# edwinyosorahardjo/compressjs-flattened

Hardware: AMD Instinct MI355X
Metric: bzip2 -9 compress MB/s at 1/2/4/8 MI355X; bit-exact output size vs ref (higher is better)
Workload: dtype u32; 1 GPU; Bzip2.compressFile level 9 (899981-byte blocks) on 1 x 100000000 bytes enwik8-shaped synthetic text (tools/textgen.c seed 1), device-resident; per_gpu_bytes=100000000, level=9, parallelism=1 GPU

## Files before the change

### compressjs-flattened_amd/csrc/bwt.hip

```cpp
#include "cjs_internal.h"
#include "prims.hpp"
#include <stdlib.h>
#include <string.h>

namespace cjs {

struct Geom { uint32_t nb, stride, n_last; };
__device__ __forceinline__ uint32_t blk_len(const Geom& g, uint32_t blk) { return blk == g.nb - 1 ? g.n_last : g.stride; }
struct VarGeom { uint32_t nb, stride, n_last; const uint32_t* len; };
__device__ __forceinline__ uint32_t blk_len(const VarGeom& g, uint32_t blk) { return g.len[blk]; }
template <typename G> struct is_var_geom { static constexpr bool value = false; };
template <> struct is_var_geom<VarGeom> { static constexpr bool value = true; };

__device__ __forceinline__ uint32_t xcd_tile(uint32_t wg, uint32_t T) {
  const uint32_t per = (T + 7u) >> 3;
  return (wg & 7u) * per + (wg >> 3);
}
__host__ __device__ __forceinline__ uint32_t xcd_grid(uint32_t T) { return ((T + 7u) >> 3) << 3; }

struct SegGeom { uint32_t nseg, stride, n_last, tps; };
struct TileRef { uint32_t seg, off, nvalid; uint64_t base; };
__device__ __forceinline__ TileRef tile_ref(const SegGeom& sg, uint32_t tile) {
  TileRef t;
  t.seg = tile / sg.tps;
// ... 351 lines not shown
    uint32_t any = 0;
    for (int j = 0; j < 8; j++) any |= hword[threadIdx.x * 8 + j];
    if (!any) atomicOr(big_flag, 1u);
  }
  surv = block_sum<256>(surv, sm);
  heads = block_sum<256>(heads, sm);
  last = wave_max(last);
  if (lane_id() == 0) sm[wave_id()] = last;
  __syncthreads();
  if (threadIdx.x == 0) {
    uint32_t m = sm[0]; for (int i = 1; i < 4; i++) m = sm[i] > m ? sm[i] : m;
    tile_cnt[blockIdx.x] = surv; tile_cnt[T + blockIdx.x] = heads; tile_cnt[2 * (size_t)T + blockIdx.x] = m;
  }
}

__global__ __launch_bounds__(1024) void bwt_scan_tiles(uint32_t* __restrict__ tile_cnt, uint32_t T, uint32_t* __restrict__ counters,
                                                      uint32_t* __restrict__ host_mirror ) {
  __shared__ uint32_t sm[16];
  __shared__ uint32_t mx[1024];
  uint32_t c0 = 0, c1 = 0, cm = 0;
  for (uint32_t base = 0; base < T; base += 1024) {
    const uint32_t i = base + threadIdx.x;
    const bool ok = i < T;
    uint32_t t0, t1;
    const uint32_t v0 = ok ? tile_cnt[i] : 0u, v1 = ok ? tile_cnt[T + i] : 0u, v2 = ok ? tile_cnt[2 * (size_t)T + i] : 0u;
    const uint32_t e0 = block_excl_sum<1024>(v0, sm, t0);
    const uint32_t e1 = block_excl_sum<1024>(v1, sm, t1);
    const uint32_t im = block_incl_max<1024>(v2, sm);
    mx[threadIdx.x] = im;
    __syncthreads();
// ... 21 lines not shown
  uint64_t lo = seg0, hi = base - 64u;
  while (hi > lo) {
    const uint64_t len = hi - lo, step = (len + 63u) / 64u, idx = lo + (uint64_t)lane * step;
    const bool hit = idx >= hi || (key[idx] >> shift) == target;
    const uint64_t hits = __ballot(hit);
    const uint32_t j = hits ? (uint32_t)__builtin_ctzll(hits) : 64u;
    if (!j) { hi = lo; break; }
    const uint64_t nhi = lo + (uint64_t)j * step;
    lo += (uint64_t)(j - 1u) * step + 1u;
    if (j < 64u && nhi < hi) hi = nhi;
  }
  return hi;
}

template <bool FIRST, bool PACKED, int SWEEP = 0, typename G = Geom>
__global__ __launch_bounds__(256) void bwt_apply(const uint64_t* __restrict__ key, const uint32_t* __restrict__ val,
                                                 const uint32_t* __restrict__ pos, uint32_t A, G g,
                                                 uint32_t* tile_cnt, uint32_t T,
                                                 uint32_t* __restrict__ R, uint32_t* __restrict__ SA,
                                                 uint32_t* __restrict__ nval, uint32_t* __restrict__ npos, uint32_t* __restrict__ ngord, HalfMap hm_,
                                                 const uint8_t* __restrict__ Tx, uint8_t* __restrict__ U, uint32_t* __restrict__ big_flag,
                                                 int gs1 , int carried ) {
  __shared__ uint64_t sk[RS_TILE + 2];
  __shared__ uint64_t m_nh[64], m_sg[64], m_oh[64];
  __shared__ uint32_t wp_s[64], wp_h[64], wp_head[64];
  __shared__ uint32_t carry_s;
  const uint32_t tile = xcd_tile(blockIdx.x, T), half = SWEEP == 2 ? 1u : 0u;
  if (tile >= T) return;
  const uint32_t hsplit = hm_.stride >> 1;
  const int tid = threadIdx.x, w = tid >> 6, lane = tid & 63;
  const uint64_t base = (uint64_t)tile * RS_TILE;
  const uint32_t nvalid = (uint32_t)((uint64_t)A - base < RS_TILE ? (uint64_t)A - base : RS_TILE);
  uint32_t sbase = 0, hbase = 0, carry = 0;
  if (SWEEP != 1) { sbase = tile_cnt[tile]; hbase = tile_cnt[T + tile]; carry = tile_cnt[2 * (size_t)T + tile]; }
  else if (w == 0) {
    const uint64_t seg0 = (uint64_t)((uint32_t)base / g.stride) * g.stride;
    const uint32_t c = (uint32_t)class_head_before(key, seg0, base, gs1, lane) + 1u;
    if (lane == 0) carry_s = c;
  }
  uint32_t p16[FIRST ? 1 : 16], v16[PACKED ? 1 : 16];
  {
    uint64_t k16[16];
#pragma unroll
    for (int it = 0; it < 16; it++) {
      const uint32_t e = (uint32_t)it * 256u + tid;
      k16[it] = __builtin_nontemporal_load(key + base + (e < nvalid ? e : nvalid - 1u));
    }
    if (!FIRST) {
#pragma unroll
      for (int it = 0; it < 16; it++) { const uint32_t e = (uint32_t)it * 256u + tid; p16[it] = __builtin_nontemporal_load(pos + base + (e < nvalid ? e : nvalid - 1u)); }
    }
    if (!PACKED) {
#pragma unroll
      for (int it = 0; it < 16; it++) { const uint32_t e = (uint32_t)it * 256u + tid; v16[it] = __builtin_nontemporal_load(val + base + (e < nvalid ? e : nvalid - 1u)); }
    }
    if (tid == 0) sk[0] = base ? key[base - 1] : ~0ull;
    if (tid == 64) sk[RS_TILE + 1] = base + RS_TILE < A ? key[base + RS_TILE] : ~0ull;
#pragma unroll
    for (int it = 0; it < 16; it++) {
      const uint32_t e = (uint32_t)it * 256u + tid;
      sk[e + 1] = e < nvalid ? k16[it] : ~0ull;
    }
  }
  __syncthreads();
  const int GS = FIRST ? gs1 : 0;
  const uint64_t bnd = FIRST ? (base + g.stride - 1u) / g.stride * g.stride : ~0ull;
#pragma unroll 4
  for (int it = 0; it < 16; it++) {
    const uint32_t e = (uint32_t)it * 256u + tid;
    const uint64_t a = base + e;
    const bool ok = e < nvalid;
    const uint64_t k = sk[e + 1] >> GS;
    const bool nh = ok && (a == 0 || a == bnd || (sk[e] >> GS) != k);
    const bool nx = a + 1 == A || a + 1 == bnd || (sk[e + 2] >> GS) != k;
    const uint64_t mnh = __ballot(nh), msg = __ballot(nh && nx);
    if (lane == 0) { m_nh[it * 4 + w] = mnh; m_sg[it * 4 + w] = msg; }
    if (!FIRST) {
      const bool oh = ok && (a == 0 || (sk[e] >> 20) != (sk[e + 1] >> 20));
      const uint64_t moh = __ballot(oh);
      if (lane == 0) m_oh[it * 4 + w] = moh;
    }
  }
  __syncthreads();
  if (w == 0) {
    const uint64_t mh = m_nh[lane], ms = m_sg[lane];
    const uint32_t first = (uint32_t)lane * 64u;
    const uint32_t nv = nvalid > first ? (nvalid - first < 64u ? nvalid - first : 64u) : 0u;
    const uint64_t vm = nv == 64 ? ~0ull : ((1ull << nv) - 1ull);
    const uint32_t sv = (uint32_t)__popcll(vm & ~ms), hd = (uint32_t)__popcll(mh & ~ms);
    const uint32_t lastrel = mh ? first + 63u - (uint32_t)__builtin_clzll(mh) + 1u : 0u;
    const uint32_t is = wave_incl_sum(sv), ih = wave_incl_sum(hd), im = wave_incl_max(lastrel);
    uint32_t em = __shfl_up(im, 1, 64);
    if (lane == 0) em = 0;
    wp_s[lane] = is - sv; wp_h[lane] = ih - hd; wp_head[lane] = em;
    if (SWEEP == 1 && lane == 63) {
      tile_cnt[tile] = is; tile_cnt[T + tile] = ih; tile_cnt[2 * (size_t)T + tile] = im ? (uint32_t)base + im : 0u;
    }
    if (SWEEP == 1) {
      const uint64_t nz = __ballot(mh != 0);
      bool bad = false;
#pragma unroll
      for (int b = 0; b < 8; b++) bad |= base + (uint64_t)(b + 1) * 512u <= A && ((nz >> (8 * b)) & 0xFFull) == 0;
      if (bad && lane == 0) atomicOr(big_flag, 1u);
// ... 21 lines not shown
  for (int it = 0; it < 16; it++) {
    const uint32_t e = (uint32_t)it * 256u + tid;
    if (e < nvalid) {
      const uint64_t a = base + e;
      const int wi = it * 4 + w;
      const uint64_t mh = m_nh[wi], ms = m_sg[wi];
      const uint64_t hm = mh & le;
      uint32_t head_a;
      bool keeps_rank = false;
      if (hm || wp_head[wi]) {
        const uint32_t hrel = hm ? (uint32_t)wi * 64u + 63u - (uint32_t)__builtin_clzll(hm) : wp_head[wi] - 1u;
        head_a = (uint32_t)base + hrel;
        if (!FIRST) keeps_rank = (m_oh[hrel >> 6] >> (hrel & 63u)) & 1ull;
      } else {
        head_a = carry - 1u;
        if (!FIRST) keeps_rank = head_a == 0 || (key[head_a] >> 20) != (key[head_a - 1] >> 20);
      }
      const uint32_t p = FIRST ? (uint32_t)a : p16[FIRST ? 0 : it];
      const uint32_t vraw = PACKED ? (uint32_t)sk[e + 1] : v16[PACKED ? 0 : it];
      const uint32_t vv = vraw & PK_POS_MASK;
      const uint32_t pb = PACKED ? (vraw >> PK2_PREV_SHIFT) & 0xFFu : vraw >> VAL_PREV_SHIFT;
      const uint32_t blk = p / g.stride;
      const uint32_t head_pos = p - ((uint32_t)a - head_a);
      if (!keeps_rank && (SWEEP == 0 || (uint32_t)(vv >= hsplit) == half)) R[(size_t)blk * g.stride + vv] = head_pos - blk * g.stride;
      if (SWEEP == 1) continue;
      if ((ms >> lane) & 1ull) {
        if (U) U[p] = (uint8_t)(carried ? pb : ub[it]);
        else __builtin_nontemporal_store(vv, SA + p);
      } else {
        const uint32_t so = sbase + wp_s[wi] + (uint32_t)__popcll(~ms & lt);
        const uint32_t ho = hbase + wp_h[wi] + (uint32_t)__popcll(mh & ~ms & le);
// ... 51 lines not shown
    else if (j >= n) { j = 0; past |= 1u << s; }
    pp[s] = blk * tg.g.stride + j;
  }
#pragma unroll
  for (int s = 0; s < 16; s++) rk20[s] = tg.R[((need >> s) & 1u) ? pp[s] : pp[0]];
#pragma unroll
  for (int s = 0; s < 16; s++) rk20[s] = ((past >> s) & 1u) ? 0u : rk20[s] + 1u;
}

__device__ __forceinline__ void ts_ce(uint64_t& a, uint64_t& b, bool up) {
  const bool sw = (a > b) == up;
  const uint64_t x = sw ? b : a, y = sw ? a : b;
  a = x; b = y;
}
template <typename TG>
__global__ __launch_bounds__(256) void bwt_tile_sort(uint64_t* __restrict__ key, uint32_t* __restrict__ val, uint32_t A,
                                                     uint8_t* __restrict__ dflag, TG tg, uint32_t Tt) {
  __shared__ uint64_t sk[TS_WIN];
  __shared__ uint64_t hm[64];
  __shared__ int32_t wlast[64], wnext[64];
  uint32_t* gk = (uint32_t*)sk;
  const int tid = threadIdx.x, w = tid >> 6, lane = tid & 63;
  __shared__ uint32_t lired[4];
  const uint32_t win = xcd_tile(blockIdx.x, Tt);
  if (win >= Tt) return;
  const uint64_t wb = (uint64_t)win * TS_NOM;
  const uint64_t we = (wb + TS_WIN < A) ? wb + TS_WIN : A;
  const uint32_t L = (uint32_t)(we - wb);
  uint64_t r[16];
  uint32_t pv[16], go[16], pp[16];
  uint32_t gprev;
// ... 69 lines not shown
    }
  }
  __syncthreads();
  uint32_t* sk32 = reinterpret_cast<uint32_t*>(sk);
#pragma unroll
  for (int it = 0; it < 16; it++) { const uint32_t x = (uint32_t)it * 256u + tid; sk32[x] = ((uint32_t)(r[it] >> 32) << 12) | x; }
  any_medium = __syncthreads_or(any_medium);
#pragma unroll
  for (int it = 0; it < 16; it++) {
    const bool own = hx16[it] != 0xFFFFFFFFu && (hx16[it] >> 16) <= TS_TINY;
    const uint32_t hx = own ? (hx16[it] & 0xFFFFu) : 0u, g = own ? (hx16[it] >> 16) : 0u;
    const uint32_t gmax = wave_max(g);
    if (gmax == 0) continue;
    const uint64_t mine = r[it];
    const uint32_t mine32 = ((uint32_t)(mine >> 32) << 12) | ((uint32_t)it * 256u + tid);
    uint32_t rank = 0;
    for (uint32_t d = 0; d < gmax; d++) rank += (d < g && sk32[hx + d] < mine32) ? 1u : 0u;
    if (own) {
      key[wb + hx + rank] = ((uint64_t)go[it] << 20) | ((mine >> 32) & 0xFFFFFull);
      val[wb + hx + rank] = (uint32_t)mine;
    }
  }
  if (!any_medium) return;
  if (w == 0) {
    const uint32_t pc = (uint32_t)__builtin_popcountll(mm[lane]);
    const uint32_t inc = wave_incl_sum(pc);
    mpre[lane] = inc - pc;
    if (lane == 63) mpre[64] = inc;
  }
  __syncthreads();
  const uint32_t Mt = mpre[64];
  uint32_t P = 2;
  while (P < Mt) P <<= 1;
  uint32_t cix[16];
// ... 24 lines not shown
      const uint32_t hj = j >> 1;
      for (uint32_t t = tid; t < (P >> 2); t += 256) {
        const uint32_t i0 = ((t & ~(hj - 1)) << 2) | (t & (hj - 1));
        const bool up = (i0 & kk) == 0;
        uint64_t e0 = sk[i0], e1 = sk[i0 | hj], e2 = sk[i0 | j], e3 = sk[i0 | j | hj];
        ts_ce(e0, e2, up); ts_ce(e1, e3, up); ts_ce(e0, e1, up); ts_ce(e2, e3, up);
        sk[i0] = e0; sk[i0 | hj] = e1; sk[i0 | j] = e2; sk[i0 | j | hj] = e3;
      }
      __syncthreads();
    }
  }
#pragma unroll
  for (int it = 0; it < 16; it++) {
    if (cix[it] != 0xFFFFFFFFu) {
      const uint32_t x = (uint32_t)it * 256u + tid;
      const uint64_t e = sk[cix[it]];
      key[wb + x] = ((uint64_t)go[it] << 20) | ((e >> 32) & 0xFFFFFull);
      val[wb + x] = (uint32_t)e;
    }
  }
}
template <typename TG>
__global__ __launch_bounds__(256) void bwt_tile_sort_radix(uint64_t* __restrict__ key, uint32_t* __restrict__ val, uint32_t A,
                                                           uint8_t* __restrict__ dflag, TG tg, uint32_t Tt) {
  __shared__ uint64_t se[TS_WIN];
  __shared__ uint64_t hm[64];
  __shared__ int32_t wlast[64], wnext[64];
  __shared__ uint32_t wcnt[4][256];
  __shared__ uint32_t sm[4];
  uint32_t* gk = (uint32_t*)se;
  const int tid = threadIdx.x, w = tid >> 6, lane = tid & 63;
  __shared__ uint32_t lired[4];
  const uint32_t win = xcd_tile(blockIdx.x, Tt);
  if (win >= Tt) return;
  const uint64_t wb = (uint64_t)win * TS_NOM;
  const uint64_t we = (wb + TS_WIN < A) ? wb + TS_WIN : A;
  const uint32_t L = (uint32_t)(we - wb);
  uint32_t rk20[16], go[16], pv[16], pp[16];
// ... 82 lines not shown
      const uint32_t d = (comp[s] >> shift) & 255u;
      se[wcnt[w][d] + rk[s]] = ((uint64_t)comp[s] << 32) | pv[s];
    }
    __syncthreads();
#pragma unroll
    for (int s = 0; s < 16; s++) {
      const uint64_t e = se[(uint32_t)w * 1024u + (uint32_t)s * 64u + lane];
      comp[s] = (uint32_t)(e >> 32); pv[s] = (uint32_t)e;
    }
    __syncthreads();
  }
#pragma unroll
  for (int s = 0; s < 16; s++) {
    if ((ownm >> s) & 1u) {
      const uint32_t x = (uint32_t)w * 1024u + (uint32_t)s * 64u + lane;
      key[wb + x] = ((uint64_t)go[s] << 20) | (comp[s] & 0xFFFFFu);
      val[wb + x] = pv[s];
    }
  }
}
__global__ __launch_bounds__(1024) void scan_u32_single(uint32_t* __restrict__ arr, uint32_t n, uint32_t* __restrict__ total, uint32_t* __restrict__ host_total) {
  __shared__ uint32_t sm[16];
  uint32_t carry = 0;
  for (uint32_t base = 0; base < n; base += 1024) {
    const uint32_t i = base + threadIdx.x;
    uint32_t v = i < n ? arr[i] : 0u, tot;
    const uint32_t ex = block_excl_sum<1024>(v, sm, tot);
    if (i < n) arr[i] = carry + ex;
    carry += tot;
  }
  if (threadIdx.x == 0) { *total = carry; *host_total = carry; }
// ... 35 lines not shown
                                                        uint64_t* __restrict__ dk, uint32_t* __restrict__ dv, uint32_t* __restrict__ dpos) {
  __shared__ uint32_t sm[4];
  const uint64_t a0 = (uint64_t)blockIdx.x * TS_GT + (uint32_t)threadIdx.x * 8u;
  uint32_t f, heads; uint64_t k8[8];
  defer_flags(A, dflag, key, a0, f, heads, k8);
  uint32_t tot;
  uint32_t o = tcount[blockIdx.x] + block_excl_sum<256>((uint32_t)__builtin_popcount(f), sm, tot);
  uint32_t hid = hcount[blockIdx.x] + block_excl_sum<256>((uint32_t)__builtin_popcount(heads), sm, tot);
#pragma unroll
  for (int j = 0; j < 8; j++) if ((f >> j) & 1u) {
    hid += (heads >> j) & 1u;
    dk[o] = ((uint64_t)(hid - 1u) << 20) | (k8[j] & 0xFFFFFull); dv[o] = val[a0 + j]; dpos[o] = (uint32_t)(a0 + j); o++;
  }
}
__global__ __launch_bounds__(256) void bwt_defer_scatter(uint32_t D, const uint64_t* __restrict__ dk, const uint32_t* __restrict__ dv,
                                                         const uint32_t* __restrict__ dpos, uint64_t* __restrict__ key, uint32_t* __restrict__ val) {
  for (uint64_t j = (uint64_t)blockIdx.x * 256 + threadIdx.x; j < D; j += (uint64_t)gridDim.x * 256) {
    const uint32_t a = dpos[j];
    key[a] = (key[a] & ~0xFFFFFull) | (dk[j] & 0xFFFFFull); val[a] = dv[j];
  }
}

template <typename G>
__global__ __launch_bounds__(256) void bwt_flush_active(uint32_t A, const uint32_t* __restrict__ val, const uint32_t* __restrict__ pos,
                                                        uint32_t* __restrict__ SA, G g, const uint8_t* __restrict__ Tx, uint8_t* __restrict__ U, int carried) {
  for (uint64_t a = (uint64_t)blockIdx.x * 256 + threadIdx.x; a < A; a += (uint64_t)gridDim.x * 256) {
    const uint32_t p = pos[a], v = val[a] & PK_POS_MASK;
    if (U && carried) U[p] = (uint8_t)(val[a] >> VAL_PREV_SHIFT);
    else if (U) { const uint32_t blk = p / g.stride; U[p] = Tx[(size_t)blk * g.stride + (v ? v - 1u : blk_len(g, blk) - 1u)]; }
    else SA[p] = v;
  }
}

__global__ __launch_bounds__(256) void bwt_phase2_records(const uint64_t* __restrict__ key, SegGeom sg, const uint8_t* __restrict__ T,
// ... 108 lines not shown
    const uint8_t* t = T + (size_t)blk * g.stride;
    uint8_t* u = U + (size_t)blk * g.stride;
    const uint32_t s = __builtin_nontemporal_load(SA + a);
    const uint32_t p0 = R[(size_t)blk * g.stride];
    if (p == p0) u[0] = t[n - 1];
    else u[p < p0 ? p + 1 : p] = t[s - 1];
  }
}

static int bits_for(uint64_t x) { int b = 0; while (x) { b++; x >>= 1; } return b; }
size_t BwtWork::bytes_needed(size_t cap) {
  const size_t T = hist_tiles_for(cap);
  size_t b = 0;
  auto add = [&](size_t n) { b += (n + 255) & ~(size_t)255; };
  add(cap * 8); add(cap * 8); add(cap * 4); add(cap * 4); add(cap * 4); add(cap * 4); add(cap * 4);
  add(cap * 4); add(cap * 4); add(cap);
  add(hist_words(T) * 4); add(256 * segs_for(cap) * 4); add(3 * T * 4); add(64); add(16 * 256 * 4);
  return b + 4096;
}
int BwtWork::carve(Arena& a, size_t cap_) {
  cap = cap_;
  const size_t T = hist_tiles_for(cap);
  hist_tiles = (uint32_t)T; bintot_segs = (uint32_t)segs_for(cap);
  key[0] = a.take<uint64_t>(cap); key[1] = a.take<uint64_t>(cap);
  val[0] = a.take<uint32_t>(cap); val[1] = a.take<uint32_t>(cap);
  pos[0] = a.take<uint32_t>(cap); pos[1] = a.take<uint32_t>(cap);
  gord = a.take<uint32_t>(cap);
  R = a.take<uint32_t>(cap); SA = a.take<uint32_t>(cap); dflag = a.take<uint8_t>(cap);
  hist = a.take<uint32_t>(hist_words(T)); bintot = a.take<uint32_t>(256 * (size_t)bintot_segs);
  tile_cnt = a.take<uint32_t>(3 * T); counters = a.take<uint32_t>(16);
  ghist = a.take<uint32_t>(16 * 256);
  if (!counters || !ghist) return CJS_E_OUT_OF_MEMORY;
  if (!h_counters) CJS_HIP_TRY(hipHostMalloc((void**)h_counters.put(), 64));
  if (!ev_scan) CJS_HIP_TRY(hipEventCreateWithFlags(ev_scan.put(), hipEventDisableTiming));
  return 0;
}

template <typename K>
static int radix_passes(hipStream_t s, BwtWork& w, K* k0, uint32_t* v0, K* k1, uint32_t* v1, int& cur, uint32_t n, int lo_bit, int hi_bit,
                        LaunchTimes* lt, const SegGeom* seg = nullptr, const GenSrc* gen = nullptr, bool noval = false,
                        bool first_hist_ready = false,
                        uint8_t* dig = nullptr) {
  const uint32_t T1 = (n + RS_TILE - 1) / RS_TILE;
// ... 35 lines not shown
}

template <typename K>
int radix_passes_public(hipStream_t s, BwtWork& w, K* k0, uint32_t* v0, K* k1, uint32_t* v1, int& cur, uint32_t n, int lo_bit, int hi_bit) {
  return radix_passes<K>(s, w, k0, v0, k1, v1, cur, n, lo_bit, hi_bit, nullptr);
}
template int radix_passes_public<uint32_t>(hipStream_t, BwtWork&, uint32_t*, uint32_t*, uint32_t*, uint32_t*, int&, uint32_t, int, int);
template <typename K>
int radix_pass_segments_public(hipStream_t s, BwtWork& w, K* k0, uint32_t* v0, K* k1, uint32_t* v1, int& cur, uint32_t nseg, uint32_t stride, int lo_bit, int hi_bit, bool noval, bool first_hist_ready) {
  const SegGeom sg{nseg, stride, stride, (stride + RS_TILE - 1) / RS_TILE};
  return radix_passes<K>(s, w, k0, v0, k1, v1, cur, nseg * stride, lo_bit, hi_bit, nullptr, &sg, nullptr, noval, first_hist_ready);
}
template int radix_pass_segments_public<uint32_t>(hipStream_t, BwtWork&, uint32_t*, uint32_t*, uint32_t*, uint32_t*, int&, uint32_t, uint32_t, int, int, bool, bool);

template <typename TG>
static void launch_tile_sort(hipStream_t s, uint32_t Tt, uint64_t* key, uint32_t* val, uint32_t A, uint8_t* dflag, uint32_t ngroups, const TG& tg) {
  if (ngroups && A / ngroups >= 5) hipLaunchKernelGGL(bwt_tile_sort_radix<TG>, dim3(xcd_grid(Tt)), dim3(256), 0, s, key, val, A, dflag, tg, Tt);
  else hipLaunchKernelGGL(bwt_tile_sort<TG>, dim3(xcd_grid(Tt)), dim3(256), 0, s, key, val, A, dflag, tg, Tt);
}
static bool tile_sorted_round(uint32_t A) { return A >= 2 * TS_WIN; }
template <typename TG>
static int sort_round(hipStream_t s, BwtWork& w, int& c, int pc, uint32_t A, int bits, LaunchTimes* lt, uint32_t ngroups, const TG& tg) {
  if (!tile_sorted_round(A)) return radix_passes<uint64_t>(s, w, w.key[0], w.val[0], w.key[1], w.val[1], c, A, 0, bits, lt);
  const uint32_t Tt = (A + TS_NOM - 1) / TS_NOM, Tg = (A + TS_GT - 1) / TS_GT;
  uint8_t* dflag = w.dflag;
  uint32_t* tcount = w.tile_cnt;
  if (w.no_large_groups) {
    launch_tile_sort(s, Tt, w.key[c], w.val[c], A, nullptr, ngroups, tg);
    CJS_HIP_TRY(hipGetLastError());
    return 0;
  }
  dev_fill(s, dflag, 1, A);
  launch_tile_sort(s, Tt, w.key[c], w.val[c], A, dflag, ngroups, tg);
  uint32_t* hcount = w.hist;
  hipLaunchKernelGGL(bwt_defer_count, dim3(Tg), dim3(256), 0, s, A, dflag, w.key[c], tcount, hcount);
  hipLaunchKernelGGL(scan_u32_single, dim3(1), dim3(1024), 0, s, hcount, Tg, w.counters + 3, w.h_counters + 3);
  hipLaunchKernelGGL(scan_u32_single, dim3(1), dim3(1024), 0, s, tcount, Tg, w.counters + 2, w.h_counters + 2);
  CJS_HIP_TRY(hipStreamSynchronize(s));
  const uint32_t D = w.h_counters[2];
  if (env_debug()) fprintf(stderr, "[cjs bwt]   tile sort: %u of %u suffixes in groups > %u\n", D, A, TS_MAXGRP);
  if (D == 0) w.no_large_groups = true;
  if (D == 0) return 0;
  if ((size_t)D > w.cap / 2) return radix_passes<uint64_t>(s, w, w.key[0], w.val[0], w.key[1], w.val[1], c, A, 0, bits, lt);
  uint64_t* dk0 = w.key[1 - c]; uint64_t* dk1 = dk0 + w.cap / 2;
  uint32_t* dv0 = w.val[1 - c]; uint32_t* dv1 = dv0 + w.cap / 2;
  uint32_t* dpos = w.pos[1 - pc];
  hipLaunchKernelGGL(bwt_defer_gather, dim3(Tg), dim3(256), 0, s, w.key[c], w.val[c], A, dflag, tcount, hcount, dk0, dv0, dpos);
  int cur = 0;
  const uint32_t ndg = w.h_counters[3];
  CJS_TRY((radix_passes<uint64_t>(s, w, dk0, dv0, dk1, dv1, cur, D, 0, 20 + bits_for(ndg ? ndg - 1 : 0), lt)));
  hipLaunchKernelGGL(bwt_defer_scatter, dim3((D + 255) / 256 < 8192u ? (D + 255) / 256 : 8192u), dim3(256), 0, s, D, cur ? dk1 : dk0, cur ? dv1 : dv0, dpos,
                     w.key[c], w.val[c]);
  CJS_HIP_TRY(hipGetLastError());
  return 0;
}

template <typename G>
static int bwt_run_impl(hipStream_t s, BwtWork& w, const uint8_t* d_T, const G g, bool cyclic, uint8_t* d_U, uint32_t* d_pidx,
                        cjs_stats* stats, bool resolve_stats) {
  constexpr bool VAR = is_var_geom<G>::value;
  const uint32_t nb = g.nb, stride = g.stride, n_last = g.n_last;
  if (nb == 0) return 0;
  if (VAR && (!cyclic || n_last != stride)) return CJS_E_INVALID_ARG;
  const uint64_t M64 = (uint64_t)(nb - 1) * stride + n_last;
  if (M64 > w.cap || M64 >= 0xFFFFF000ull) return CJS_E_INVALID_ARG;
  if (stride > (1u << 20) - 2) return CJS_E_INVALID_ARG;
  const uint32_t M = (uint32_t)M64;
// ... 25 lines not shown
  const int gs1 = packed ? PK2_GSHIFT : 0;
  const int carried = packed ? 1 : 0;
  for (;;) {
    if (rounds == 0) {
      if (packed) {
        CJS_TRY((radix_passes<uint64_t>(s, w, w.key[0], w.val[0], w.key[1], w.val[1], c, A, PK_KEY_LO, 64, &lt, &sg, &gen, true, false, w.dflag)));
        hipLaunchKernelGGL(bwt_phase2_records, dim3(sg.nseg * sg.tps), dim3(256), 0, s, w.key[c], sg, d_T, w.hist, w.key[1 - c]);
        c = 1 - c;
        CJS_TRY((radix_passes<uint64_t>(s, w, w.key[0], w.val[0], w.key[1], w.val[1], c, A, 48, 64, &lt, &sg, nullptr, true, true, w.dflag)));
      } else if (segmented) CJS_TRY((radix_passes<uint64_t>(s, w, w.key[0], w.val[0], w.key[1], w.val[1], c, A, 0, bits, &lt, &sg, &gen)));
      else CJS_TRY((radix_passes<uint64_t>(s, w, w.key[0], w.val[0], w.key[1], w.val[1], c, A, 0, bits, &lt)));
    } else CJS_TRY(sort_round(s, w, c, pc, A, bits, &lt, ngroups, tg));
    const uint32_t T = (A + RS_TILE - 1) / RS_TILE;
    if (rounds == 0 && sweeps) {
      const HalfMap hm{2u, stride};
      hipLaunchKernelGGL((bwt_apply<true, true, 1, G>), dim3(xcd_grid(T)), dim3(256), 0, s, w.key[c], w.val[c], w.pos[pc], A, g, w.tile_cnt, T, w.R, w.SA,
                         w.val[1 - c], w.pos[1 - pc], w.gord, hm, dT, dU, w.counters + 4, gs1, carried);
      hipLaunchKernelGGL(bwt_scan_tiles, dim3(1), dim3(1024), 0, s, w.tile_cnt, T, w.counters, w.h_counters);
      CJS_HIP_TRY(hipEventRecord(w.ev_scan, s));
      hipLaunchKernelGGL((bwt_apply<true, true, 2, G>), dim3(xcd_grid(T)), dim3(256), 0, s, w.key[c], w.val[c], w.pos[pc], A, g, w.tile_cnt, T, w.R, w.SA,
                         w.val[1 - c], w.pos[1 - pc], w.gord, hm, dT, dU, w.counters + 4, gs1, carried);
    } else {
    hipLaunchKernelGGL(bwt_flags, dim3(T), dim3(256), 0, s, w.key[c], A, w.tile_cnt, T, rounds == 0 ? gs1 : 0, w.counters + 4, rounds == 0 ? stride : 0u);
    hipLaunchKernelGGL(bwt_scan_tiles, dim3(1), dim3(1024), 0, s, w.tile_cnt, T, w.counters, w.h_counters);
    CJS_HIP_TRY(hipEventRecord(w.ev_scan, s));
    if (rounds == 0) {
      const HalfMap hm{1u, stride};
      const uint32_t grid = xcd_grid(T);
      if (packed) hipLaunchKernelGGL((bwt_apply<true, true, 0, G>), dim3(grid), dim3(256), 0, s, w.key[c], w.val[c], w.pos[pc], A, g, w.tile_cnt, T, w.R, w.SA,
                                     w.val[1 - c], w.pos[1 - pc], w.gord, hm, dT, dU, w.counters + 4, gs1, carried);
      else hipLaunchKernelGGL((bwt_apply<true, false, 0, G>), dim3(grid), dim3(256), 0, s, w.key[c], w.val[c], w.pos[pc], A, g, w.tile_cnt, T, w.R, w.SA,
                              w.val[1 - c], w.pos[1 - pc], w.gord, hm, dT, dU, w.counters + 4, gs1, carried);
    } else hipLaunchKernelGGL((bwt_apply<false, false, 0, G>), dim3(xcd_grid(T)), dim3(256), 0, s, w.key[c], w.val[c], w.pos[pc], A, g, w.tile_cnt, T, w.R, w.SA,
                              w.val[1 - c], w.pos[1 - pc], w.gord, HalfMap{1u, stride}, dT, dU, w.counters + 4, gs1, carried);
    }
    CJS_HIP_TRY(hipEventSynchronize(w.ev_scan));
    rounds++;
    const uint32_t A2 = w.h_counters[0], NG = w.h_counters[1];
    if (w.h_counters[4] == 0) w.no_large_groups = true;
    if (env_debug()) fprintf(stderr, "[cjs bwt] round %u h=%u A=%u bits=%d -> A'=%u groups=%u\n", rounds, h, A, bits, A2, NG);
    c = 1 - c; pc = 1 - pc;
    A = A2; ngroups = NG;
    if (A == 0) break;
    if (cyclic && h >= max_n) {
      hipLaunchKernelGGL(bwt_flush_active<G>, dim3((A + 255) / 256), dim3(256), 0, s, A, w.val[c], w.pos[pc], w.SA, g, dT, dU, carried);
      break;
    }
    if (rounds > 40) return CJS_E_HIP;
// ... 34 lines not shown
```

### compressjs-flattened_amd/csrc/cjs_internal.h

```cpp
#pragma once
#include <hip/hip_runtime.h>
#include <stdint.h>
#include <stddef.h>
#include <stdio.h>
#include <new>
#include "cjs_hip.h"

#define CJS_HIP_TRY(expr)                                                                   \
  do {                                                                                      \
    hipError_t _e = (expr);                                                                 \
    if (_e != hipSuccess) {                                                                 \
      fprintf(stderr, "[cjs_hip] %s failed: %s (%s:%d)\n", #expr, hipGetErrorString(_e), __FILE__, __LINE__); \
      return _e == hipErrorOutOfMemory ? CJS_E_OUT_OF_MEMORY : CJS_E_HIP;                    \
    }                                                                                       \
  } while (0)
#define CJS_TRY(expr) do { int _rc = (expr); if (_rc) return _rc; } while (0)

namespace cjs {

void clear_detail();
void set_detail(const char* fmt, ...);
bool env_debug(); bool env_no_ctx_cache();

#define CJS_GUARD_BEGIN try {
// ... 114 lines not shown
    }
    for (int i = 2 * n; i < made; i++) (void)hipEventDestroy(ev[i]);
    n = made = 0;
  }
};

struct BwtWork {
  size_t cap = 0;
  uint64_t* key[2] = {nullptr, nullptr};
  uint32_t* val[2] = {nullptr, nullptr};
  uint32_t* pos[2] = {nullptr, nullptr};
  uint32_t* gord = nullptr;
  uint32_t* R = nullptr;
  uint32_t* SA = nullptr;
  uint8_t* dflag = nullptr;
  uint32_t* hist = nullptr;
  uint32_t* bintot = nullptr;
  uint32_t* tile_cnt = nullptr;
  uint32_t* counters = nullptr;
  uint32_t* ghist = nullptr;
  Pinned<uint32_t> h_counters;
  Event ev_scan;
  uint32_t hist_tiles = 0, bintot_segs = 0;
  LaunchTimes lt;
  bool no_large_groups = false;
  static size_t hist_tiles_for(size_t cap) { return (cap + RS_TILE - 1) / RS_TILE + cap / 65536 + 258; }
  static size_t segs_for(size_t cap) { return cap / 65536 + 2; }
  static size_t hist_words(size_t tiles) { return 256 * (tiles + tiles / 64 + 2); }
  static size_t bytes_needed(size_t cap);
  int carve(Arena& a, size_t cap);
// ... 14 lines not shown
```

Baseline: 8632 MB/s.

## Replace 64-bit key reloads with per-suffix byte head flags in BWT refinement rounds

The sort kernels (tile sort, radix tile sort, defer scatter, and a new whole-sort flag kernel) now write a one-byte flag per suffix marking a new key group and a new old-rank group, instead of writing back 64-bit composite keys. Later rounds' tile counting and apply kernels read these packed flags (16 per thread as uint4) in place of 8-byte keys, and build the head and singleton bitmasks from them. This cuts global memory traffic and shared memory use in the non-first rounds. In exchange it adds a cap-sized flag buffer, an extra flag kernel after whole-array radix sorts, and a key gather on the large-deferred fallback path, with more complex rank/equality logic in the tile sorts.

Measured after the change: 9080 MB/s (median of 6 runs). +5.2%, better.

```diff
diff --git a/compressjs-flattened_amd/csrc/bwt.hip b/compressjs-flattened_amd/csrc/bwt.hip
--- a/compressjs-flattened_amd/csrc/bwt.hip
+++ b/compressjs-flattened_amd/csrc/bwt.hip
@@ -389,6 +389,64 @@
   }
 }
 
+constexpr uint32_t HF_NEW = 1u, HF_OLD = 2u;
+__device__ __forceinline__ uint32_t hf_bits16(const uint4& v, int bit) {
+  const uint32_t M = 0x01020408u;
+  const uint32_t n0 = (((v.x >> bit) & 0x01010101u) * M) >> 24, n1 = (((v.y >> bit) & 0x01010101u) * M) >> 24;
+  const uint32_t n2 = (((v.z >> bit) & 0x01010101u) * M) >> 24, n3 = (((v.w >> bit) & 0x01010101u) * M) >> 24;
+  return (n0 & 15u) | ((n1 & 15u) << 4) | ((n2 & 15u) << 8) | ((n3 & 15u) << 12);
+}
+__device__ __forceinline__ uint4 hf_load16(const uint8_t* __restrict__ hflag, uint64_t base, uint32_t nvalid, int tid, uint32_t& valid) {
+  const uint32_t first = (uint32_t)tid * 16u;
+  const uint32_t nv = nvalid > first ? (nvalid - first < 16u ? nvalid - first : 16u) : 0u;
+  valid = (1u << nv) - 1u;
+  uint4 v = make_uint4(0u, 0u, 0u, 0u);
+  if (nv) v = *reinterpret_cast<const uint4*>(hflag + base + first);
+  return v;
+}
+__global__ __launch_bounds__(256) void bwt_key_flags(const uint64_t* __restrict__ key, uint32_t A, uint8_t* __restrict__ hflag) {
+  for (uint64_t a = (uint64_t)blockIdx.x * 256 + threadIdx.x; a < A; a += (uint64_t)gridDim.x * 256) {
+    const uint64_t k = key[a], p = a ? key[a - 1] : ~k;
+    hflag[a] = (uint8_t)((k != p ? HF_NEW : 0u) | ((k >> 20) != (p >> 20) ? HF_OLD : 0u));
+  }
+}
+__global__ __launch_bounds__(256) void bwt_flags_bytes(const uint8_t* __restrict__ hflag, uint32_t A, uint32_t* __restrict__ tile_cnt, uint32_t T,
+                                                       uint32_t* __restrict__ big_flag) {
+  __shared__ uint32_t nhs[257];
+  __shared__ uint32_t sm[4];
+  const int tid = threadIdx.x;
+  const uint64_t base = (uint64_t)blockIdx.x * RS_TILE;
+  const uint32_t nvalid = (uint32_t)((uint64_t)A - base < RS_TILE ? (uint64_t)A - base : RS_TILE);
+  uint32_t valid;
+  const uint4 v = hf_load16(hflag, base, nvalid, tid, valid);
+  const uint32_t nh = hf_bits16(v, 0) & valid;
+  nhs[tid] = nh | (~valid & 0xFFFFu);
+  if (tid == 0) nhs[256] = base + RS_TILE < A ? (uint32_t)hflag[base + RS_TILE] & HF_NEW : 1u;
+  __syncthreads();
+  const uint32_t nx = ((nhs[tid] >> 1) | (nhs[tid + 1] << 15)) & 0xFFFFu;
+  const uint32_t single = nh & nx;
+  uint32_t surv = (uint32_t)__popc(valid & ~single), heads = (uint32_t)__popc(nh & ~single);
+  uint32_t last = nh ? (uint32_t)base + (uint32_t)tid * 16u + 32u - (uint32_t)__clz(nh) : 0u;
+  {
+    const uint64_t any = __ballot(nh != 0);
+    const uint32_t run0 = (uint32_t)wave_id() * 2u;
+    if (lane_id() == 0) {
+      bool bad = false;
+      for (uint32_t b = 0; b < 2; b++) bad |= base + (uint64_t)(run0 + b + 1u) * 512u <= A && (uint32_t)(any >> (32 * b)) == 0u;
+      if (bad) atomicOr(big_flag, 1u);
+    }
+  }
+  surv = block_sum<256>(surv, sm);
+  heads = block_sum<256>(heads, sm);
+  last = wave_max(last);
+  if (lane_id() == 0) sm[wave_id()] = last;
+  __syncthreads();
+  if (tid == 0) {
+    uint32_t m = sm[0]; for (int i = 1; i < 4; i++) m = sm[i] > m ? sm[i] : m;
+    tile_cnt[blockIdx.x] = surv; tile_cnt[T + blockIdx.x] = heads; tile_cnt[2 * (size_t)T + blockIdx.x] = m;
+  }
+}
+
 __global__ __launch_bounds__(1024) void bwt_scan_tiles(uint32_t* __restrict__ tile_cnt, uint32_t T, uint32_t* __restrict__ counters,
                                                       uint32_t* __restrict__ host_mirror ) {
   __shared__ uint32_t sm[16];
@@ -440,17 +498,18 @@
 }
 
 template <bool FIRST, bool PACKED, int SWEEP = 0, typename G = Geom>
-__global__ __launch_bounds__(256) void bwt_apply(const uint64_t* __restrict__ key, const uint32_t* __restrict__ val,
+__global__ __launch_bounds__(256) void bwt_apply(const uint64_t* __restrict__ key , const uint8_t* __restrict__ hflag ,
+                                                 const uint32_t* __restrict__ val,
                                                  const uint32_t* __restrict__ pos, uint32_t A, G g,
                                                  uint32_t* tile_cnt, uint32_t T,
                                                  uint32_t* __restrict__ R, uint32_t* __restrict__ SA,
                                                  uint32_t* __restrict__ nval, uint32_t* __restrict__ npos, uint32_t* __restrict__ ngord, HalfMap hm_,
                                                  const uint8_t* __restrict__ Tx, uint8_t* __restrict__ U, uint32_t* __restrict__ big_flag,
                                                  int gs1 , int carried ) {
-  __shared__ uint64_t sk[RS_TILE + 2];
+  __shared__ uint64_t sk[FIRST ? RS_TILE + 2 : 1];
   __shared__ uint64_t m_nh[64], m_sg[64], m_oh[64];
   __shared__ uint32_t wp_s[64], wp_h[64], wp_head[64];
-  __shared__ uint32_t carry_s;
+  __shared__ uint32_t carry_s, nx_s;
   const uint32_t tile = xcd_tile(blockIdx.x, T), half = SWEEP == 2 ? 1u : 0u;
   if (tile >= T) return;
   const uint32_t hsplit = hm_.stride >> 1;
@@ -466,53 +525,69 @@
   }
   uint32_t p16[FIRST ? 1 : 16], v16[PACKED ? 1 : 16];
   {
-    uint64_t k16[16];
-#pragma unroll
+    uint64_t k16[FIRST ? 16 : 1];
+    uint4 hv = make_uint4(0u, 0u, 0u, 0u);
+    uint32_t hvalid = 0;
+    if constexpr (FIRST) {
+#pragma unroll
+      for (int it = 0; it < 16; it++) {
+        const uint32_t e = (uint32_t)it * 256u + tid;
+        k16[it] = __builtin_nontemporal_load(key + base + (e < nvalid ? e : nvalid - 1u));
+      }
+    } else hv = hf_load16(hflag, base, nvalid, tid, hvalid);
+    if (!FIRST) {
+#pragma unroll
+      for (int it = 0; it < 16; it++) { const uint32_t e = (uint32_t)it * 256u + tid; p16[it] = __builtin_nontemporal_load(pos + base + (e < nvalid ? e : nvalid - 1u)); }
+    }
+    if (!PACKED) {
+#pragma unroll
+      for (int it = 0; it < 16; it++) { const uint32_t e = (uint32_t)it * 256u + tid; v16[it] = __builtin_nontemporal_load(val + base + (e < nvalid ? e : nvalid - 1u)); }
+    }
+    if constexpr (FIRST) {
+      if (tid == 0) sk[0] = base ? key[base - 1] : ~0ull;
+      if (tid == 64) sk[RS_TILE + 1] = base + RS_TILE < A ? key[base + RS_TILE] : ~0ull;
+#pragma unroll
+      for (int it = 0; it < 16; it++) {
+        const uint32_t e = (uint32_t)it * 256u + tid;
+        sk[e + 1] = e < nvalid ? k16[it] : ~0ull;
+      }
+    } else {
+      reinterpret_cast<uint16_t*>(m_nh)[tid] = (uint16_t)(hf_bits16(hv, 0) & hvalid);
+      reinterpret_cast<uint16_t*>(m_oh)[tid] = (uint16_t)(hf_bits16(hv, 1) & hvalid);
+      if (tid == 64) nx_s = base + RS_TILE < A ? (uint32_t)hflag[base + RS_TILE] & HF_NEW : 1u;
+    }
+  }
+  __syncthreads();
+  if constexpr (FIRST) {
+    const int GS = gs1;
+    const uint64_t bnd = (base + g.stride - 1u) / g.stride * g.stride;
+#pragma unroll 4
     for (int it = 0; it < 16; it++) {
       const uint32_t e = (uint32_t)it * 256u + tid;
-      k16[it] = __builtin_nontemporal_load(key + base + (e < nvalid ? e : nvalid - 1u));
-    }
-    if (!FIRST) {
-#pragma unroll
-      for (int it = 0; it < 16; it++) { const uint32_t e = (uint32_t)it * 256u + tid; p16[it] = __builtin_nontemporal_load(pos + base + (e < nvalid ? e : nvalid - 1u)); }
-    }
-    if (!PACKED) {
-#pragma unroll
-      for (int it = 0; it < 16; it++) { const uint32_t e = (uint32_t)it * 256u + tid; v16[it] = __builtin_nontemporal_load(val + base + (e < nvalid ? e : nvalid - 1u)); }
-    }
-    if (tid == 0) sk[0] = base ? key[base - 1] : ~0ull;
-    if (tid == 64) sk[RS_TILE + 1] = base + RS_TILE < A ? key[base + RS_TILE] : ~0ull;
-#pragma unroll
-    for (int it = 0; it < 16; it++) {
-      const uint32_t e = (uint32_t)it * 256u + tid;
-      sk[e + 1] = e < nvalid ? k16[it] : ~0ull;
-    }
-  }
-  __syncthreads();
-  const int GS = FIRST ? gs1 : 0;
-  const uint64_t bnd = FIRST ? (base + g.stride - 1u) / g.stride * g.stride : ~0ull;
-#pragma unroll 4
-  for (int it = 0; it < 16; it++) {
-    const uint32_t e = (uint32_t)it * 256u + tid;
-    const uint64_t a = base + e;
-    const bool ok = e < nvalid;
-    const uint64_t k = sk[e + 1] >> GS;
-    const bool nh = ok && (a == 0 || a == bnd || (sk[e] >> GS) != k);
-    const bool nx = a + 1 == A || a + 1 == bnd || (sk[e + 2] >> GS) != k;
-    const uint64_t mnh = __ballot(nh), msg = __ballot(nh && nx);
-    if (lane == 0) { m_nh[it * 4 + w] = mnh; m_sg[it * 4 + w] = msg; }
-    if (!FIRST) {
-      const bool oh = ok && (a == 0 || (sk[e] >> 20) != (sk[e + 1] >> 20));
-      const uint64_t moh = __ballot(oh);
-      if (lane == 0) m_oh[it * 4 + w] = moh;
-    }
-  }
-  __syncthreads();
+      const uint64_t a = base + e;
+      const bool ok = e < nvalid;
+      const uint64_t k = sk[e + 1] >> GS;
+      const bool nh = ok && (a == 0 || a == bnd || (sk[e] >> GS) != k);
+      const bool nx = a + 1 == A || a + 1 == bnd || (sk[e + 2] >> GS) != k;
+      const uint64_t mnh = __ballot(nh), msg = __ballot(nh && nx);
+      if (lane == 0) { m_nh[it * 4 + w] = mnh; m_sg[it * 4 + w] = msg; }
+    }
+    __syncthreads();
+  }
   if (w == 0) {
-    const uint64_t mh = m_nh[lane], ms = m_sg[lane];
+    const uint64_t mh = m_nh[lane];
     const uint32_t first = (uint32_t)lane * 64u;
     const uint32_t nv = nvalid > first ? (nvalid - first < 64u ? nvalid - first : 64u) : 0u;
     const uint64_t vm = nv == 64 ? ~0ull : ((1ull << nv) - 1ull);
+    uint64_t ms;
+    if constexpr (FIRST) ms = m_sg[lane];
+    else {
+      const uint64_t mhx = mh | ~vm;
+      uint32_t nb = __shfl_down((uint32_t)(mhx & 1ull), 1, 64);
+      if (lane == 63) nb = nx_s;
+      ms = mh & ((mhx >> 1) | ((uint64_t)nb << 63));
+      m_sg[lane] = ms;
+    }
     const uint32_t sv = (uint32_t)__popcll(vm & ~ms), hd = (uint32_t)__popcll(mh & ~ms);
     const uint32_t lastrel = mh ? first + 63u - (uint32_t)__builtin_clzll(mh) + 1u : 0u;
     const uint32_t is = wave_incl_sum(sv), ih = wave_incl_sum(hd), im = wave_incl_max(lastrel);
@@ -564,7 +639,7 @@
         if (!FIRST) keeps_rank = (m_oh[hrel >> 6] >> (hrel & 63u)) & 1ull;
       } else {
         head_a = carry - 1u;
-        if (!FIRST) keeps_rank = head_a == 0 || (key[head_a] >> 20) != (key[head_a - 1] >> 20);
+        if (!FIRST) keeps_rank = (hflag[head_a] & HF_OLD) != 0;
       }
       const uint32_t p = FIRST ? (uint32_t)a : p16[FIRST ? 0 : it];
       const uint32_t vraw = PACKED ? (uint32_t)sk[e + 1] : v16[PACKED ? 0 : it];
@@ -646,7 +721,7 @@
   a = x; b = y;
 }
 template <typename TG>
-__global__ __launch_bounds__(256) void bwt_tile_sort(uint64_t* __restrict__ key, uint32_t* __restrict__ val, uint32_t A,
+__global__ __launch_bounds__(256) void bwt_tile_sort(uint64_t* __restrict__ key, uint32_t* __restrict__ val, uint8_t* __restrict__ hflag, uint32_t A,
                                                      uint8_t* __restrict__ dflag, TG tg, uint32_t Tt) {
   __shared__ uint64_t sk[TS_WIN];
   __shared__ uint64_t hm[64];
@@ -746,10 +821,15 @@
     if (gmax == 0) continue;
     const uint64_t mine = r[it];
     const uint32_t mine32 = ((uint32_t)(mine >> 32) << 12) | ((uint32_t)it * 256u + tid);
-    uint32_t rank = 0;
-    for (uint32_t d = 0; d < gmax; d++) rank += (d < g && sk32[hx + d] < mine32) ? 1u : 0u;
+    uint32_t rank = 0, same = 0;
+    for (uint32_t d = 0; d < gmax; d++) {
+      const uint32_t o = sk32[hx + d];
+      const bool lt = d < g && o < mine32;
+      rank += lt ? 1u : 0u;
+      same += (lt && (o >> 12) == (mine32 >> 12)) ? 1u : 0u;
+    }
     if (own) {
-      key[wb + hx + rank] = ((uint64_t)go[it] << 20) | ((mine >> 32) & 0xFFFFFull);
+      hflag[wb + hx + rank] = (uint8_t)((same ? 0u : HF_NEW) | (rank ? 0u : HF_OLD));
       val[wb + hx + rank] = (uint32_t)mine;
     }
   }
@@ -804,14 +884,15 @@
   for (int it = 0; it < 16; it++) {
     if (cix[it] != 0xFFFFFFFFu) {
       const uint32_t x = (uint32_t)it * 256u + tid;
-      const uint64_t e = sk[cix[it]];
-      key[wb + x] = ((uint64_t)go[it] << 20) | ((e >> 32) & 0xFFFFFull);
+      const uint32_t c = cix[it];
+      const uint64_t e = sk[c], pe = c ? sk[c - 1] : ~e;
+      hflag[wb + x] = (uint8_t)(((e >> 32) != (pe >> 32) ? HF_NEW : 0u) | ((e >> 52) != (pe >> 52) ? HF_OLD : 0u));
       val[wb + x] = (uint32_t)e;
     }
   }
 }
 template <typename TG>
-__global__ __launch_bounds__(256) void bwt_tile_sort_radix(uint64_t* __restrict__ key, uint32_t* __restrict__ val, uint32_t A,
+__global__ __launch_bounds__(256) void bwt_tile_sort_radix(uint64_t* __restrict__ key, uint32_t* __restrict__ val, uint8_t* __restrict__ hflag, uint32_t A,
                                                            uint8_t* __restrict__ dflag, TG tg, uint32_t Tt) {
   __shared__ uint64_t se[TS_WIN];
   __shared__ uint64_t hm[64];
@@ -924,7 +1005,8 @@
   for (int s = 0; s < 16; s++) {
     if ((ownm >> s) & 1u) {
       const uint32_t x = (uint32_t)w * 1024u + (uint32_t)s * 64u + lane;
-      key[wb + x] = ((uint64_t)go[s] << 20) | (comp[s] & 0xFFFFFu);
+      const uint32_t pc = x ? (uint32_t)(se[x - 1] >> 32) : ~comp[s];
+      hflag[wb + x] = (uint8_t)((comp[s] != pc ? HF_NEW : 0u) | ((comp[s] >> 20) != (pc >> 20) ? HF_OLD : 0u));
       val[wb + x] = pv[s];
     }
   }
@@ -990,10 +1072,11 @@
   }
 }
 __global__ __launch_bounds__(256) void bwt_defer_scatter(uint32_t D, const uint64_t* __restrict__ dk, const uint32_t* __restrict__ dv,
-                                                         const uint32_t* __restrict__ dpos, uint64_t* __restrict__ key, uint32_t* __restrict__ val) {
+                                                         const uint32_t* __restrict__ dpos, uint8_t* __restrict__ hflag, uint32_t* __restrict__ val) {
   for (uint64_t j = (uint64_t)blockIdx.x * 256 + threadIdx.x; j < D; j += (uint64_t)gridDim.x * 256) {
     const uint32_t a = dpos[j];
-    key[a] = (key[a] & ~0xFFFFFull) | (dk[j] & 0xFFFFFull); val[a] = dv[j];
+    const uint64_t k = dk[j], p = j ? dk[j - 1] : ~k;
+    hflag[a] = (uint8_t)((k != p ? HF_NEW : 0u) | ((k >> 20) != (p >> 20) ? HF_OLD : 0u)); val[a] = dv[j];
   }
 }
 
@@ -1132,7 +1215,7 @@
   size_t b = 0;
   auto add = [&](size_t n) { b += (n + 255) & ~(size_t)255; };
   add(cap * 8); add(cap * 8); add(cap * 4); add(cap * 4); add(cap * 4); add(cap * 4); add(cap * 4);
-  add(cap * 4); add(cap * 4); add(cap);
+  add(cap * 4); add(cap * 4); add(cap); add(cap);
   add(hist_words(T) * 4); add(256 * segs_for(cap) * 4); add(3 * T * 4); add(64); add(16 * 256 * 4);
   return b + 4096;
 }
@@ -1144,7 +1227,7 @@
   val[0] = a.take<uint32_t>(cap); val[1] = a.take<uint32_t>(cap);
   pos[0] = a.take<uint32_t>(cap); pos[1] = a.take<uint32_t>(cap);
   gord = a.take<uint32_t>(cap);
-  R = a.take<uint32_t>(cap); SA = a.take<uint32_t>(cap); dflag = a.take<uint8_t>(cap);
+  R = a.take<uint32_t>(cap); SA = a.take<uint32_t>(cap); dflag = a.take<uint8_t>(cap); hflag = a.take<uint8_t>(cap);
   hist = a.take<uint32_t>(hist_words(T)); bintot = a.take<uint32_t>(256 * (size_t)bintot_segs);
   tile_cnt = a.take<uint32_t>(3 * T); counters = a.take<uint32_t>(16);
   ghist = a.take<uint32_t>(16 * 256);
@@ -1210,24 +1293,30 @@
 template int radix_pass_segments_public<uint32_t>(hipStream_t, BwtWork&, uint32_t*, uint32_t*, uint32_t*, uint32_t*, int&, uint32_t, uint32_t, int, int, bool, bool);
 
 template <typename TG>
-static void launch_tile_sort(hipStream_t s, uint32_t Tt, uint64_t* key, uint32_t* val, uint32_t A, uint8_t* dflag, uint32_t ngroups, const TG& tg) {
-  if (ngroups && A / ngroups >= 5) hipLaunchKernelGGL(bwt_tile_sort_radix<TG>, dim3(xcd_grid(Tt)), dim3(256), 0, s, key, val, A, dflag, tg, Tt);
-  else hipLaunchKernelGGL(bwt_tile_sort<TG>, dim3(xcd_grid(Tt)), dim3(256), 0, s, key, val, A, dflag, tg, Tt);
+static void launch_tile_sort(hipStream_t s, uint32_t Tt, uint64_t* key, uint32_t* val, uint8_t* hflag, uint32_t A, uint8_t* dflag, uint32_t ngroups, const TG& tg) {
+  if (ngroups && A / ngroups >= 5) hipLaunchKernelGGL(bwt_tile_sort_radix<TG>, dim3(xcd_grid(Tt)), dim3(256), 0, s, key, val, hflag, A, dflag, tg, Tt);
+  else hipLaunchKernelGGL(bwt_tile_sort<TG>, dim3(xcd_grid(Tt)), dim3(256), 0, s, key, val, hflag, A, dflag, tg, Tt);
+}
+static int sort_round_whole(hipStream_t s, BwtWork& w, int& c, uint32_t A, int bits, LaunchTimes* lt) {
+  CJS_TRY((radix_passes<uint64_t>(s, w, w.key[0], w.val[0], w.key[1], w.val[1], c, A, 0, bits, lt)));
+  hipLaunchKernelGGL(bwt_key_flags, dim3((A + 255) / 256 < 8192u ? (A + 255) / 256 : 8192u), dim3(256), 0, s, w.key[c], A, w.hflag);
+  CJS_HIP_TRY(hipGetLastError());
+  return 0;
 }
 static bool tile_sorted_round(uint32_t A) { return A >= 2 * TS_WIN; }
 template <typename TG>
 static int sort_round(hipStream_t s, BwtWork& w, int& c, int pc, uint32_t A, int bits, LaunchTimes* lt, uint32_t ngroups, const TG& tg) {
-  if (!tile_sorted_round(A)) return radix_passes<uint64_t>(s, w, w.key[0], w.val[0], w.key[1], w.val[1], c, A, 0, bits, lt);
+  if (!tile_sorted_round(A)) return sort_round_whole(s, w, c, A, bits, lt);
   const uint32_t Tt = (A + TS_NOM - 1) / TS_NOM, Tg = (A + TS_GT - 1) / TS_GT;
   uint8_t* dflag = w.dflag;
   uint32_t* tcount = w.tile_cnt;
   if (w.no_large_groups) {
-    launch_tile_sort(s, Tt, w.key[c], w.val[c], A, nullptr, ngroups, tg);
+    launch_tile_sort(s, Tt, w.key[c], w.val[c], w.hflag, A, nullptr, ngroups, tg);
     CJS_HIP_TRY(hipGetLastError());
     return 0;
   }
   dev_fill(s, dflag, 1, A);
-  launch_tile_sort(s, Tt, w.key[c], w.val[c], A, dflag, ngroups, tg);
+  launch_tile_sort(s, Tt, w.key[c], w.val[c], w.hflag, A, dflag, ngroups, tg);
   uint32_t* hcount = w.hist;
   hipLaunchKernelGGL(bwt_defer_count, dim3(Tg), dim3(256), 0, s, A, dflag, w.key[c], tcount, hcount);
   hipLaunchKernelGGL(scan_u32_single, dim3(1), dim3(1024), 0, s, hcount, Tg, w.counters + 3, w.h_counters + 3);
@@ -1237,7 +1326,11 @@
   if (env_debug()) fprintf(stderr, "[cjs bwt]   tile sort: %u of %u suffixes in groups > %u\n", D, A, TS_MAXGRP);
   if (D == 0) w.no_large_groups = true;
   if (D == 0) return 0;
-  if ((size_t)D > w.cap / 2) return radix_passes<uint64_t>(s, w, w.key[0], w.val[0], w.key[1], w.val[1], c, A, 0, bits, lt);
+  if ((size_t)D > w.cap / 2) {
+    const uint32_t Tk = (A + RS_TILE - 1) / RS_TILE;
+    hipLaunchKernelGGL(bwt_gather_keys<decltype(tg.g)>, dim3(xcd_grid(Tk)), dim3(256), 0, s, tg.g, tg.cyclic, A, tg.h, tg.R, w.val[c], tg.pos, tg.gord, w.key[c], Tk);
+    return sort_round_whole(s, w, c, A, bits, lt);
+  }
   uint64_t* dk0 = w.key[1 - c]; uint64_t* dk1 = dk0 + w.cap / 2;
   uint32_t* dv0 = w.val[1 - c]; uint32_t* dv1 = dv0 + w.cap / 2;
   uint32_t* dpos = w.pos[1 - pc];
@@ -1246,7 +1339,7 @@
   const uint32_t ndg = w.h_counters[3];
   CJS_TRY((radix_passes<uint64_t>(s, w, dk0, dv0, dk1, dv1, cur, D, 0, 20 + bits_for(ndg ? ndg - 1 : 0), lt)));
   hipLaunchKernelGGL(bwt_defer_scatter, dim3((D + 255) / 256 < 8192u ? (D + 255) / 256 : 8192u), dim3(256), 0, s, D, cur ? dk1 : dk0, cur ? dv1 : dv0, dpos,
-                     w.key[c], w.val[c]);
+                     w.hflag, w.val[c]);
   CJS_HIP_TRY(hipGetLastError());
   return 0;
 }
@@ -1302,24 +1395,25 @@
     const uint32_t T = (A + RS_TILE - 1) / RS_TILE;
     if (rounds == 0 && sweeps) {
       const HalfMap hm{2u, stride};
-      hipLaunchKernelGGL((bwt_apply<true, true, 1, G>), dim3(xcd_grid(T)), dim3(256), 0, s, w.key[c], w.val[c], w.pos[pc], A, g, w.tile_cnt, T, w.R, w.SA,
+      hipLaunchKernelGGL((bwt_apply<true, true, 1, G>), dim3(xcd_grid(T)), dim3(256), 0, s, w.key[c], nullptr, w.val[c], w.pos[pc], A, g, w.tile_cnt, T, w.R, w.SA,
                          w.val[1 - c], w.pos[1 - pc], w.gord, hm, dT, dU, w.counters + 4, gs1, carried);
       hipLaunchKernelGGL(bwt_scan_tiles, dim3(1), dim3(1024), 0, s, w.tile_cnt, T, w.counters, w.h_counters);
       CJS_HIP_TRY(hipEventRecord(w.ev_scan, s));
-      hipLaunchKernelGGL((bwt_apply<true, true, 2, G>), dim3(xcd_grid(T)), dim3(256), 0, s, w.key[c], w.val[c], w.pos[pc], A, g, w.tile_cnt, T, w.R, w.SA,
+      hipLaunchKernelGGL((bwt_apply<true, true, 2, G>), dim3(xcd_grid(T)), dim3(256), 0, s, w.key[c], nullptr, w.val[c], w.pos[pc], A, g, w.tile_cnt, T, w.R, w.SA,
                          w.val[1 - c], w.pos[1 - pc], w.gord, hm, dT, dU, w.counters + 4, gs1, carried);
     } else {
-    hipLaunchKernelGGL(bwt_flags, dim3(T), dim3(256), 0, s, w.key[c], A, w.tile_cnt, T, rounds == 0 ? gs1 : 0, w.counters + 4, rounds == 0 ? stride : 0u);
+    if (rounds == 0) hipLaunchKernelGGL(bwt_flags, dim3(T), dim3(256), 0, s, w.key[c], A, w.tile_cnt, T, gs1, w.counters + 4, stride);
+    else hipLaunchKernelGGL(bwt_flags_bytes, dim3(T), dim3(256), 0, s, w.hflag, A, w.tile_cnt, T, w.counters + 4);
     hipLaunchKernelGGL(bwt_scan_tiles, dim3(1), dim3(1024), 0, s, w.tile_cnt, T, w.counters, w.h_counters);
     CJS_HIP_TRY(hipEventRecord(w.ev_scan, s));
     if (rounds == 0) {
       const HalfMap hm{1u, stride};
       const uint32_t grid = xcd_grid(T);
-      if (packed) hipLaunchKernelGGL((bwt_apply<true, true, 0, G>), dim3(grid), dim3(256), 0, s, w.key[c], w.val[c], w.pos[pc], A, g, w.tile_cnt, T, w.R, w.SA,
+      if (packed) hipLaunchKernelGGL((bwt_apply<true, true, 0, G>), dim3(grid), dim3(256), 0, s, w.key[c], nullptr, w.val[c], w.pos[pc], A, g, w.tile_cnt, T, w.R, w.SA,
                                      w.val[1 - c], w.pos[1 - pc], w.gord, hm, dT, dU, w.counters + 4, gs1, carried);
-      else hipLaunchKernelGGL((bwt_apply<true, false, 0, G>), dim3(grid), dim3(256), 0, s, w.key[c], w.val[c], w.pos[pc], A, g, w.tile_cnt, T, w.R, w.SA,
+      else hipLaunchKernelGGL((bwt_apply<true, false, 0, G>), dim3(grid), dim3(256), 0, s, w.key[c], nullptr, w.val[c], w.pos[pc], A, g, w.tile_cnt, T, w.R, w.SA,
                               w.val[1 - c], w.pos[1 - pc], w.gord, hm, dT, dU, w.counters + 4, gs1, carried);
-    } else hipLaunchKernelGGL((bwt_apply<false, false, 0, G>), dim3(xcd_grid(T)), dim3(256), 0, s, w.key[c], w.val[c], w.pos[pc], A, g, w.tile_cnt, T, w.R, w.SA,
+    } else hipLaunchKernelGGL((bwt_apply<false, false, 0, G>), dim3(xcd_grid(T)), dim3(256), 0, s, nullptr, w.hflag, w.val[c], w.pos[pc], A, g, w.tile_cnt, T, w.R, w.SA,
                               w.val[1 - c], w.pos[1 - pc], w.gord, HalfMap{1u, stride}, dT, dU, w.counters + 4, gs1, carried);
     }
     CJS_HIP_TRY(hipEventSynchronize(w.ev_scan));
diff --git a/compressjs-flattened_amd/csrc/cjs_internal.h b/compressjs-flattened_amd/csrc/cjs_internal.h
--- a/compressjs-flattened_amd/csrc/cjs_internal.h
+++ b/compressjs-flattened_amd/csrc/cjs_internal.h
@@ -152,6 +152,7 @@
   uint32_t* R = nullptr;
   uint32_t* SA = nullptr;
   uint8_t* dflag = nullptr;
+  uint8_t* hflag = nullptr;
   uint32_t* hist = nullptr;
   uint32_t* bintot = nullptr;
   uint32_t* tile_cnt = nullptr;
```
